# cielavenir/7bgzf

Hardware: AMD Instinct MI355X
Metric: GB/s input compressed, BGZF 64KiB blocks (higher is better)
Workload: dtype u8

## Files before the change

7bgzf_amd/csrc/hd_deflate_static.hpp:

```cpp
#pragma once
#include <type_traits>
#include "hd_device.hpp"

namespace hd {

constexpr uint32_t HD_HINT_NO_WHOLE = 1;
constexpr uint32_t HD_HINT_NO_SEG = 2;
constexpr uint32_t BESIDE_KEEP_MAX = 3;

struct DeflateArgs {
	const uint8_t *in;
	const uint64_t *in_off;
	const uint32_t *in_len;
	uint32_t nblocks;
	int frame;
	int level;
	uint8_t *out;
	uint64_t out_stride;
	uint32_t out_cap;
	uint32_t *out_len;
	uint32_t *crc;
	int32_t *status;
	const CrcTables *ct;
	uint8_t *scratch;
	uint32_t first;
	uint32_t count;
	uint32_t skip_small;
	uint32_t split_max;
	uint32_t *split_ovf;
	uint32_t seg_limit;
	uint32_t seg_bytes;
	uint32_t hint;
	const uint64_t *host_seg_off;
	const uint32_t *host_seg_len;
	uint32_t parts = 0;
	uint32_t seg_slots = 0;
	uint32_t *done_flag = nullptr, *done_count = nullptr;
	uint32_t done_epoch = 0;
	uint32_t wg = 0;
	uint32_t lat = 0;
	uint32_t wg_split = 0;
	const uint8_t *stage_in = nullptr;
	uint32_t *stalls = nullptr;
	uint32_t *ready = nullptr, *arrived = nullptr, *next = nullptr;
	uint32_t span_sub = 0;
	uint8_t *scratch_b = nullptr;
	uint32_t *emitted = nullptr;
	uint32_t take_sub = 0;
	uint32_t *poison = nullptr;
	uint32_t beside_keep = BESIDE_KEEP_MAX;
	uint32_t prime_max = 0;
	void *beside = nullptr;
};

__host__ __device__ __forceinline__ uint32_t frame_hdr_bytes(int frame)
{
	return frame == HD_FRAME_BGZF ? 18u : frame == HD_FRAME_MIGZ ? 20u : frame == HD_FRAME_ZLIB ? 2u
	     : frame == HD_FRAME_GZIP ? 10u : 0u;
}

__host__ __device__ __forceinline__ uint32_t frame_trl_bytes(int frame)
{
	return frame == HD_FRAME_ZLIB ? 4u : (frame == HD_FRAME_BGZF || frame == HD_FRAME_MIGZ || frame == HD_FRAME_GZIP) ? 8u : 0u;
}

__device__ __forceinline__ uint32_t frame_trl_field(int frame, uint32_t k, uint32_t crc, uint32_t n)
{
	const uint32_t w = k < 2 ? (frame == HD_FRAME_ZLIB ? 0u : crc) : n;
	return (w >> (16 * (k & 1))) & 0xffff;
}

__device__ __forceinline__ uint32_t frame_sfx_bytes(int frame)
{
	return frame == HD_FRAME_RAW_FLUSH ? 5u : 0u;
}

__host__ __device__ inline uint32_t seg_slots_per_block(uint32_t cap, uint32_t seg)
{
	const uint32_t full = HD_STORED_SIZE(seg) + 5u;
	return cap / full + (cap % full >= 11u ? 1u : 0u);
}

__host__ __device__ inline bool seg_coded(uint32_t len, uint32_t limit, uint32_t seg, int frame, uint64_t out_stride, uint32_t out_cap)
{
	if (!limit || len <= limit)
		return false;
	if (seg == HD_SEG_BYTES || len > HD_SEG_LIMIT)
		return true;
	uint64_t room = out_stride < out_cap ? out_stride : out_cap;
	const uint32_t S = seg_slots_per_block(room > 0x7fffffffu ? 0x7fffffffu : (uint32_t)room, seg);
	if (frame == HD_FRAME_BGZF && room > 65536)
		room = 65536;
	return HD_SEGN_COUNT(len, seg) <= S &&
	       frame_hdr_bytes(frame) + HD_SEGN_WORST((uint64_t)len, seg, frame == HD_FRAME_RAW_FLUSH) + frame_trl_bytes(frame) <= room;
}

__device__ __forceinline__ bool whole_refused(const DeflateArgs &a, uint32_t n)
{
	return a.level >= 1 && !a.seg_limit && n > HD_SEG_LIMIT;
}

__device__ __forceinline__ void refuse_member(const DeflateArgs &a, uint32_t b, uint32_t lane)
{
	if (lane == 0) {
		a.out_len[b] = 0;
		if (a.status) a.status[b] = 1;
		if (a.crc) a.crc[b] = 0;
	}
}

__device__ __forceinline__ uint32_t frame_hdr_word(int frame, uint32_t j)
{
	const bool bz = frame == HD_FRAME_BGZF, gz = frame == HD_FRAME_GZIP, zl = frame == HD_FRAME_ZLIB;
	const uint32_t w0 = zl ? 0x0000da78u : gz ? 0x00088b1fu : 0x04088b1fu;
	const uint32_t w2 = zl ? 0u : gz ? 0x00000002u : bz ? 0x0006ff00u : 0x0008ff00u;
	const uint32_t w3 = (zl || gz) ? 0u : bz ? 0x00024342u : 0x00045a4du;
	return j == 0 ? w0 : j == 1 ? 0u : j == 2 ? w2 : w3;
}

__device__ __forceinline__ uint32_t frame_hdr_byte(int frame, uint32_t o, uint32_t sizefield)
{
	const uint32_t w = o < 16 ? frame_hdr_word(frame, o >> 2) : sizefield;
	return (w >> (8 * (o & 3))) & 0xff;
}

__device__ __forceinline__ void write_stored_member(const DeflateArgs &a, uint32_t b, const uint8_t *src, uint32_t n,
						  uint32_t crc, uint32_t lane)
{
	const uint32_t hdr = frame_hdr_bytes(a.frame), trl = frame_trl_bytes(a.frame);
	const bool flush = a.frame == HD_FRAME_RAW_FLUSH;
	const uint32_t stored = HD_STORED_SIZE(n);
	const uint32_t total = hdr + stored + trl + (flush ? 5u : 0u);
	uint64_t cap = a.out_stride < a.out_cap ? a.out_stride : a.out_cap;
	if (a.frame == HD_FRAME_BGZF && cap > 65536)
		cap = 65536;
	if (total > cap) {
		if (lane == 0) {
			a.out_len[b] = 0;
			if (a.status) a.status[b] = 1;
			if (a.crc) a.crc[b] = crc;
		}
		return;
	}
	const uint32_t sizefield = a.frame == HD_FRAME_BGZF ? total - 1 : stored;
	const uint32_t nblk = n == 0 ? 1u : (n + 65534u) / 65535u;
	uint32_t *dst32 = (uint32_t *)(a.out + (uint64_t)b * a.out_stride);
	for (uint32_t j = lane; j < (total + 3) / 4; j += 64) {
		uint32_t w = 0;
		for (uint32_t k = 0; k < 4; k++) {
			uint32_t o = 4 * j + k, v = 0;
			if (o < hdr) {
				v = frame_hdr_byte(a.frame, o, sizefield);
			} else if (o < hdr + stored) {
				uint32_t q = (o - hdr) / 65540u, r = (o - hdr) - q * 65540u;
				uint32_t left = n - q * 65535u;
				uint32_t bl = left < 65535u ? left : 65535u;
				if (r == 0) v = (q + 1 == nblk && !flush) ? 1u : 0u;
				else if (r == 1) v = bl & 0xff;
				else if (r == 2) v = bl >> 8;
				else if (r == 3) v = ~bl & 0xff;
				else if (r == 4) v = (~bl >> 8) & 0xff;
				else v = src[q * 65535u + r - 5];
			} else if (o < total) {
				uint32_t t = o - hdr - stored;
				v = flush ? (t >= 3 ? 0xffu : 0u) : (frame_trl_field(a.frame, t >> 1, crc, n) >> (8 * (t & 1))) & 0xff;
			}
			w |= v << (8 * k);
		}
		dst32[j] = w;
	}
	if (lane == 0) {
		a.out_len[b] = total;
		if (a.status) a.status[b] = 0;
		if (a.crc) a.crc[b] = crc;
	}
}

__device__ __forceinline__ uint4 load_slot(const uint8_t *src, uint32_t n, uint32_t piece, uint32_t lane, bool aligned)
{
	const uint32_t o = piece * HD_PIECE + lane * 16;
	if (aligned && o + 16 <= n)
		return *(const uint4 *)(src + o);
	uint32_t w0 = 0, w1 = 0, w2 = 0, w3 = 0;
	if (o < n) {
#pragma unroll
		for (uint32_t k = 0; k < 4; k++) {
			w0 |= (o + k < n ? (uint32_t)src[o + k] : 0u) << (8 * k);
			w1 |= (o + 4 + k < n ? (uint32_t)src[o + 4 + k] : 0u) << (8 * k);
			w2 |= (o + 8 + k < n ? (uint32_t)src[o + 8 + k] : 0u) << (8 * k);
			w3 |= (o + 12 + k < n ? (uint32_t)src[o + 12 + k] : 0u) << (8 * k);
		}
	}
	return make_uint4(w0, w1, w2, w3);
}

struct SplitLayout {
	uint32_t cap_tok, max_db;
	uint64_t off_rec, off_ntok, off_hist, bytes;
};
__host__ __device__ inline SplitLayout split_layout(uint32_t max_block, bool full = false)
{
	SplitLayout l;
	l.cap_tok = full ? ((max_block + 64 + 15) & ~15u) : max_block / 4 * 3 + 128;
	l.max_db = l.cap_tok / HD_DYN_BLOCK_TOKENS + 2;
	l.off_rec = (uint64_t)l.cap_tok * 4;
	l.off_ntok = l.off_rec + 16;
	l.off_hist = (l.off_ntok + (uint64_t)l.max_db * 4 + 15) & ~(uint64_t)15;
	l.bytes = l.off_hist + (uint64_t)l.max_db * 320 * 4;
	return l;
}
__device__ __forceinline__ uint8_t *split_block(uint8_t *scratch, uint32_t max_block, uint32_t i)
{
	return scratch + (uint64_t)i * split_layout(max_block).bytes;
}
__host__ __device__ inline SplitLayout part_layout() { return split_layout(HD_LAT_PART_BYTES, true); }
__device__ __forceinline__ uint8_t *part_block(uint8_t *scratch, uint32_t i)
{
	return scratch + (uint64_t)i * part_layout().bytes;
}

template <int WIN_BITS, int HASH_BITS, bool TOK, int INTRA = 0, bool PRIMED = TOK>
__global__ __launch_bounds__(64) void k_deflate_static(DeflateArgs a)
{
	static_assert(PRIMED || !TOK, "the parse kernels are always built with the latency-mode paths");
	static_assert(!TOK || (WIN_BITS == HD_L2_WIN_BITS && HASH_BITS == HD_L2_HASH_BITS && HD_L2_MIN_LEN == HD_MIN_MATCH),
		      "the parse kernel is level 2's: its ring, its table, its minimum length");
	constexpr uint32_t W = 1u << WIN_BITS;
	constexpr uint32_t W4M = W / 4 - 1;
	constexpr uint32_t HS = HD_TABLE_ENTRIES(WIN_BITS, HASH_BITS);
	constexpr uint32_t STG = 64;
	constexpr uint32_t TOKQ = 128;
	constexpr bool K16 = TOK;

	__shared__ __attribute__((aligned(W))) uint32_t ring32[W / 4 + 4];
	__shared__ __attribute__((aligned(16))) uint16_t table[HS];
	__shared__ __attribute__((aligned(16))) uint32_t stage[TOK ? 316 : STG];
	__shared__ uint32_t tokbuf[TOKQ];
	const uint32_t ring_lds = (uint32_t)(uintptr_t)(__attribute__((address_space(3))) const void *)ring32;

	const uint32_t lane = threadIdx.x;
	const bool parted = PRIMED && TOK && a.parts != 0;
	const uint32_t b = a.first + (parted ? blockIdx.x / a.parts : blockIdx.x);
	if (b >= a.nblocks)
		return;
	const ClockStamp clk(TOK ? HD_CLK_PARSE : HD_CLK_STATIC);
	const uint8_t *src = a.in + a.in_off[b];
	uint32_t n = a.in_len[b];
	uint32_t prime = (PRIMED && HD_LAT_SEG_PRIME && a.seg_slots && b % a.seg_slots) ? HD_LAT_PRIME(HD_LAT_PRIME_BYTES, n) : 0u;
	if (parted) {
		const uint32_t o = (blockIdx.x % a.parts) * HD_LAT_PART_BYTES;
		if (o >= n)
			return;
		n = n - o < HD_LAT_PART_BYTES ? n - o : HD_LAT_PART_BYTES;
		prime = o ? HD_LAT_PRIME(o, n) : HD_LAT_PRIME(prime, n);
		src += o;
	}
	const uint8_t *const src_own = src;
	const uint32_t n_own = n;
	src -= prime;
	n += prime;
	if (TOK && !parted && (n > a.split_max || seg_coded(n_own, a.seg_limit, a.seg_bytes, a.frame, a.out_stride, a.out_cap))) {
		if (lane == 0)
			a.split_ovf[b] = 1;
		return;
	}
	if (!TOK && seg_coded(n_own, a.seg_limit, a.seg_bytes, a.frame, a.out_stride, a.out_cap))
		return;
	if (!TOK && whole_refused(a, n_own)) {
		refuse_member(a, b, lane);
		return;
	}
	const bool aligned = (((uintptr_t)src) & 15) == 0;
	uint32_t *dst32 = (uint32_t *)(a.out + (uint64_t)b * a.out_stride);
	const CrcTables *ct = a.ct;

	const uint32_t hdr = frame_hdr_bytes(a.frame), trl = frame_trl_bytes(a.frame);
	uint64_t cap64 = a.out_stride < a.out_cap ? a.out_stride : a.out_cap;
	if (a.frame == HD_FRAME_BGZF && cap64 > 65536)
		cap64 = 65536;
	const uint32_t cap = (uint32_t)cap64;
	const uint32_t stored = HD_STORED_SIZE(n_own);
	uint32_t limit = stored - 1;
	const bool flush = a.frame == HD_FRAME_RAW_FLUSH;
	const uint32_t sfx = frame_sfx_bytes(a.frame);
	bool use_static = TOK || (a.level >= 1 && cap >= hdr + trl + sfx + 2);
	if (!TOK && use_static && cap - hdr - trl - sfx < limit)
		limit = cap - hdr - trl - sfx;
	const uint32_t limit_bits = limit > 0x1fffffe0u ? 0xffffff00u : 8u * limit;

	for (uint32_t i = lane; i < HS / 8; i += 64)
		((uint4 *)table)[i] = make_uint4(0, 0, 0, 0);
	for (uint32_t i = lane; i < (TOK ? 316u : STG); i += 64)
		stage[i] = 0;
	if (!TOK && lane < 4 && hdr)
		stage[lane] = frame_hdr_word(a.frame, lane);
	const SplitLayout lay = parted ? part_layout() : split_layout(TOK ? a.split_max : 0);
	uint8_t *const rec = !TOK ? nullptr : parted ? part_block(a.scratch, blockIdx.x) : split_block(a.scratch, a.split_max, blockIdx.x);
	uint32_t *const slab = (uint32_t *)rec;
	uint32_t ntok_slab = 0, db_start = 0, ndb = 0;
	int32_t db_room = HD_DYN_BLOCK_TOKENS;

	Fn8Ident fid;
	fid.init(lane);
	Fn8Cross fcross;
	fcross.init(lane);
	uint32_t lane_k = lane + (HD_TOKEN_MATCH_TAG - (3u << 16));
	asm volatile("" : "+v"(lane_k));
	HashConsts hk;
	hk.init(HS);
	CrcLanes crc;
	crc.init(lane, n, prime);
	uint32_t filled = 0;
	uint4 pre = load_slot(src, n, 0, lane, aligned);

	uint32_t bitpos = 8 * hdr;
	uint32_t flushed = 0;
	const uint32_t paybase = 8 * hdr;

	auto put = [&](uint32_t code, uint32_t nbits, uint32_t incl, uint32_t total) {
		const uint32_t bp = bitpos + incl - nbits;
		const uint32_t sh = bp & 31, i = (bp >> 5) & (STG - 1);
		const uint64_t wide = (uint64_t)code << sh;
		atomicOr(&stage[i], (uint32_t)wide);
		atomicOr(&stage[(i + 1) & (STG - 1)], (uint32_t)(wide >> 32));
		bitpos += total;
	};
	auto drain_read = [&](uint32_t &fl) -> uint32_t {
		const uint32_t ready = (bitpos >> 5) - flushed;
		fl = flushed + lane;
		asm("" : "+v"(fl));
		uint32_t v;
		asm("" : "=v"(v));
		if (lane < ready) {
			const uint32_t i = fl & (STG - 1);
			v = stage[i];
			stage[i] = 0;
		}
		return v;
	};
	auto drain_store = [&](uint32_t fl, uint32_t v) {
		const uint32_t ready = (bitpos >> 5) - flushed;
		if (lane < ready)
			dst32[fl] = v;
		flushed = bitpos >> 5;
	};
	auto drain = [&]() {
		uint32_t fl;
		const uint32_t v = drain_read(fl);
		drain_store(fl, v);
	};
	auto crc_then_prefetch = [&](uint32_t piece, uint4 v) {
		crc.fold(ct, piece, piece * HD_PIECE + lane * 16 + 16 <= n && piece * HD_PIECE + lane * 16 >= prime, v);
		asm volatile("" : "+v"(crc.s) : : "memory");
		if (filled < n)
			pre = load_slot(src, n, piece + 1, lane, aligned);
	};
	auto fill_piece = [&]() {
		const uint32_t piece = filled / HD_PIECE;
		const uint4 v = pre;
		filled += HD_PIECE;
		const uint32_t ro = (piece * HD_PIECE) & (W - 1);
		((uint4 *)ring32)[ro / 16 + lane] = v;
		if (ro == 0 && lane == 0)
			((uint4 *)ring32)[W / 16] = v;
		crc_then_prefetch(piece, v);
	};
	struct Fetched {
		uint32_t v, vh, c;
	};
	constexpr bool OWN_AHEAD = false;
	struct Own {
		uint32_t w0, w1, w2;
	};
	auto own = [&](uint32_t S_) -> Own {
		const uint32_t *w = &ring32[((S_ + lane) >> 2) & W4M];
		Own o = { w[0], w[1], w[2] };
		return o;
	};
	Own o1 = { 0, 0, 0 };
	auto fetch = [&](auto inner_tag, uint32_t S_) -> Fetched {
		constexpr bool INNER = decltype(inner_tag)::value;
		Fetched f;
		const uint32_t p = S_ + lane;
		const uint32_t *w = &ring32[(p >> 2) & W4M];
		uint32_t w0, w1, w2;
		if (OWN_AHEAD && S_ >= 128) {
			w0 = o1.w0;
			w1 = o1.w1;
			w2 = o1.w2;
		} else {
			w0 = w[0];
			w1 = w[1];
			w2 = w[2];
		}
		f.v = __builtin_amdgcn_alignbyte(w1, w0, p & 3);
		f.vh = __builtin_amdgcn_alignbyte(w2, w1, p & 3);
		const bool can = INNER || p + HD_MIN_MATCH <= n;
		const uint32_t ha = hash_slot_addr(f.v, hk);
		uint16_t *const slot = (uint16_t *)((uint8_t *)table + (can ? ha : 0u));
		const uint16_t mine = (uint16_t)(p + 1);
		const uint32_t e = *slot;
		if (can)
			*slot = mine;
		if (INNER) {
			f.c = e;
		} else {
			const uint32_t back = (p + 1 - e) & 0xffffu;
			f.c = (can && e && back) ? p + 1 - back : 0u;
		}
		if (INTRA) {
			const uint32_t d = intra_step_distance<INTRA>(f.v, lane);
			f.c = (can && d) ? p + 1 - d : f.c;
		}
		return f;
	};
	struct Probed {
		uint32_t c0, c1, c2;
		uint32_t spare[10];
	};
	auto probe = [&](uint32_t c, uint32_t p) -> Probed {
		Probed q = {};
		const uint32_t *w = &ring32[((c - 1) >> 2) & W4M];
		q.c0 = w[0];
		q.c1 = w[1];
		q.c2 = w[2];
		return q;
	};

	uint32_t qhead = 0, qtail = 0;
	uint32_t Q0 = 0, qn = 0;
	uint32_t Qp = 0;
	uint64_t qpm = 0;
	auto queue_settle = [&]() {
		Q0 = sel(qpm, Qp, Q0);
		qpm = 0;
	};
	auto count_symbol = [&](uint32_t c) {
		atomicAdd(&stage[c], 1u);
	};
	auto emit_tokens = [&](uint32_t count, uint32_t tq) -> bool {
		uint32_t t = tq;
		if (TOK) {
			t = tokbuf[(qhead + lane) & (TOKQ - 1)];
			qhead += count;
		}
		if (!use_static)
			return false;
		if (TOK) {
			if (ntok_slab + count > lay.cap_tok)
				return use_static = false;
			if (lane < count) {
				slab[ntok_slab + lane] = t;
				if (t & HD_TOKEN_MATCH) {
					uint32_t ls, leb, lev, ds, deb, dev;
					len_slot(((t >> 16) & 0xff) + 3, ls, leb, lev);
					off_slot((t & 0xffff) + 1, ds, deb, dev);
					count_symbol(257 + ls);
					count_symbol(286 + ds);
				} else {
					count_symbol(t & 0xff);
				}
			}
			ntok_slab += count;
			return true;
		}
		const uint64_t mmask = __ballot((int32_t)t < 0);
		const uint64_t vmask = count >= 64 ? ~0ull : (1ull << (count & 63)) - 1;
		uint32_t e0 = ct->SL[sel(mmask, (t >> 16) & 0x1ff, t & 0xff)];
		uint32_t ds, deb, dev;
		off_slot((t & 0xffff) + 1, ds, deb, dev);
		uint32_t dpart = (__brev(ds) >> 27) | (dev << 5);
		asm volatile("" : "+v"(dpart), "+v"(deb) : : "memory");
		uint32_t fl;
		const uint32_t dv = drain_read(fl);
		asm volatile("" : "+v"(e0) : : "memory");
		drain_store(fl, dv);
		const uint32_t nb0 = e0 >> 16;
		const uint32_t code = sel(vmask, sel(mmask, (e0 & 0xffff) | (dpart << nb0), e0 & 0xffff), 0u);
		const uint32_t nbits = sel(vmask, sel(mmask, nb0 + 5 + deb, nb0), 0u);
		const uint32_t incl = wave_incl_scan<true>(nbits);
		const uint32_t total = readlane(incl, 63);
		if ((bitpos - paybase) + total + 7 > limit_bits)
			return use_static = false;
		put(code, nbits, incl, total);
		return true;
	};

	if (!TOK)
		put(lane == 0 ? (flush ? 2u : 3u) : 0u, lane == 0 ? 3u : 0u, 3u, 3u);

	Fetched f0 = { 0, 0, 0 }, f1 = { 0, 0, 0 };
	Probed q0 = {};
	if (use_static && n) {
		fill_piece();
		f0 = fetch(std::false_type{}, 0);
		q0 = probe(f0.c, lane);
		f1 = fetch(std::false_type{}, 64);
		if (OWN_AHEAD)
			o1 = own(128);
	}
	uint32_t carry = 0;
	auto step = [&](auto inner_tag, auto nofill_tag, auto room258_tag, uint32_t S) -> bool {
		constexpr bool INNER = decltype(inner_tag)::value;
		constexpr bool NOFILL = decltype(nofill_tag)::value;
		constexpr bool ROOM258 = decltype(room258_tag)::value;
		if (!NOFILL && filled < n && filled < S + HD_LOOKAHEAD)
			fill_piece();
		const uint32_t lo = filled > W ? filled - W : 0;
		const uint32_t lanes = INNER ? 64u : (n - S < 64 ? n - S : 64);

		const Fetched fc = f0;
		const Probed qc = q0;
		f0 = f1;
		q0 = probe(f1.c, S + 64 + lane);
		f1 = fetch(inner_tag, S + 128);
		if (OWN_AHEAD)
			o1 = own(S + 192);
		if (!TOK)
			queue_settle();

		const uint64_t lanem = (INNER || lanes == 64) ? ~0ull : (1ull << (lanes & 63)) - 1;
		constexpr bool GROUP = !TOK && INNER && ROOM258;
		const uint32_t p = S + (GROUP ? lane_k : lane);
		const uint32_t cv0 = fc.v, cvh0 = fc.vh;
		const uint32_t room = n - p;
		const uint32_t c = fc.c, cp = c - 1;
		const uint32_t cv = __builtin_amdgcn_alignbyte(qc.c1, qc.c0, cp);
		const uint32_t cvh = __builtin_amdgcn_alignbyte(qc.c2, qc.c1, cp);
		const uint32_t x = cvh ^ cvh0;
		const uint64_t xm = __ballot(cvh == cvh0);
		const uint32_t len8 = sel(xm, 8u, 4u + ((uint32_t)__builtin_ctz(x) >> 3));
		uint64_t okm = __ballot((int32_t)cp >= (int32_t)lo) & __ballot(cv == cv0);
		const uint32_t mylen = INNER ? len8 : (len8 < room ? len8 : room);
		if (!INNER)
			okm &= __ballot(p + HD_MIN_MATCH <= n);

		if (carry >= lanes) {
			carry -= lanes;
			return true;
		}

		const uint64_t capmask = INNER ? (okm & xm) : (okm & xm & __ballot(room > 8));
		const uint32_t jump8 = sel(okm, mylen, 1u);
		uint32_t lenv = jump8;
		const uint64_t livem = ~0ull << carry;
		const uint32_t mw_base = GROUP ? p - c : (p + (HD_TOKEN_MATCH_TAG - (3u << 16) - 1u)) - cp;
		const uint32_t lit = cv0 & 0xff;
		uint32_t len16 = 8;
		const bool k16_step = K16 && capmask != 0;
		if (k16_step) {
			const uint32_t *wp = &ring32[(p >> 2) & W4M], *wc = &ring32[(cp >> 2) & W4M];
			const uint32_t c2 = qc.c2;
			const uint32_t p2 = wp[2], p3 = wp[3], p4 = wp[4];
			const uint32_t c3 = wc[3], c4 = wc[4];
			const uint32_t xa = __builtin_amdgcn_alignbyte(p3, p2, p & 3) ^ __builtin_amdgcn_alignbyte(c3, c2, cp);
			const uint32_t xb = __builtin_amdgcn_alignbyte(p4, p3, p & 3) ^ __builtin_amdgcn_alignbyte(c4, c3, cp);
			uint32_t fa, fb;
			asm("v_ffbl_b32 %0, %1" : "=v"(fa) : "v"(xa));
			asm("v_ffbl_b32 %0, %1" : "=v"(fb) : "v"(xb));
			const uint32_t ka = (fa >> 3) < 4 ? (fa >> 3) : 4u, kb = (fb >> 3) < 4 ? (fb >> 3) : 4u;
			len16 = 8 + ka + (ka >> 2) * kb;
			if (!INNER)
				len16 = len16 < room ? len16 : room;
		}
		uint64_t k8m = 0, par = 0, contm = 0;
		uint32_t jumpA = jump8, jumpW = jump8;
		if (k16_step) {
			k8m = capmask & __ballot(len16 == 16);
			const uint64_t capk = capmask & ~k8m & __ballot(len16 != 8);
			par = capk;
			if (capk & (capk << 8)) {
#pragma unroll
				for (int i = 0; i < 7; i++)
					par = capk & ~(par << 8);
			}
			contm = (par << 8) & lanem;
			const uint32_t kc = (uint32_t)__builtin_amdgcn_ds_bpermute((int)((lane - 8) << 2), (int)(len16 - 8));
			jumpW = sel(capk, len16, jump8);
			jumpA = sel(contm, kc, jump8);
			lenv = jumpW;
		}
		uint64_t starts;
		{
			Fn8 f;
			f.lo = sel(livem, jumpA + 0x0200ffffu, 0x02010000u);
			f.hi = 0x06050403u;
			const uint32_t w0 = fn8_scan_state0(f, fid, fcross);
			starts = livem & ~(__ballot((w0 & 0xff) != 0) << 1);
		}
		uint64_t v = 0;
		if (K16) {
			uint64_t pend = ~0ull;
			for (;;) {
				v = starts & contm & ((starts & par) << 8);
				const uint64_t ev = starts & (k8m | contm) & ~v & pend;
				if (!ev)
					break;
				const uint32_t m = (uint32_t)__ffsll((unsigned long long)ev) - 1;
				uint32_t len;
				if ((k8m >> m) & 1) {
					const uint32_t pm = S + m;
					const uint32_t dm = pm + 1 - readlane(c, m);
					const uint32_t maxlen = n - pm < HD_MAX_MATCH ? n - pm : HD_MAX_MATCH;
					uint32_t t0, t1, k;
					len = 16;
					asm volatile("Lhd_ext_%=:\n\t"
					     "v_add_u32 %[t0], %[len], %[vb]\n\t"
					     "v_add_u32 %[t1], %[ndm], %[t0]\n\t"
					     "v_and_or_b32 %[t0], %[t0], %[msk], %[rb]\n\t"
					     "v_and_or_b32 %[t1], %[t1], %[msk], %[rb]\n\t"
					     "ds_read_u8 %[t0], %[t0]\n\t"
					     "ds_read_u8 %[t1], %[t1]\n\t"
					     "s_waitcnt lgkmcnt(0)\n\t"
					     "v_cmp_ne_u16 vcc, %[t0], %[t1]\n\t"
					     "s_cbranch_vccnz Lhd_ext_hit_%=\n\t"
					     "s_add_u32 %[len], %[len], 64\n\t"
					     "s_cmp_lt_u32 %[len], %[maxlen]\n\t"
					     "s_cbranch_scc1 Lhd_ext_%=\n\t"
					     "s_branch Lhd_ext_done_%=\n"
					     "Lhd_ext_hit_%=:\n\t"
					     "s_ff1_i32_b64 %[k], vcc\n\t"
					     "s_add_u32 %[len], %[len], %[k]\n"
					     "Lhd_ext_done_%=:"
					     : [len] "+s"(len), [t0] "=&v"(t0), [t1] "=&v"(t1), [k] "=&s"(k)
					     : [vb] "v"(pm + lane), [ndm] "s"(0u - dm), [msk] "s"(W - 1), [rb] "v"(ring_lds), [maxlen] "s"(maxlen)
					     : "vcc", "scc", "memory");
					len = len < maxlen ? len : maxlen;
					asm("s_mov_b32 m0, %2\n\ts_nop 0\n\tv_writelane_b32 %0, %1, m0" : "+v"(lenv) : "s"(len), "s"(m));
				} else {
					len = readlane(jumpW, m);
				}
				uint64_t fresh = 0;
				uint32_t xq = m + (uint32_t)__builtin_amdgcn_readfirstlane((int)len), hop;
				asm volatile("s_cmp_gt_u32 %0, 63\n\t"
					     "s_cbranch_scc1 Lhd_rethread_done_%=\n"
					     "Lhd_rethread_%=:\n\t"
					     "s_bitcmp1_b64 %3, %0\n\t"
					     "s_cbranch_scc1 Lhd_rethread_done_%=\n\t"
					     "s_bitset1_b64 %1, %0\n\t"
					     "v_readlane_b32 %2, %4, %0\n\t"
					     "s_add_u32 %0, %0, %2\n\t"
					     "s_cmp_lt_u32 %0, 64\n\t"
					     "s_cbranch_scc1 Lhd_rethread_%=\n"
					     "Lhd_rethread_done_%=:"
					     : "+s"(xq), "+s"(fresh), "=&s"(hop)
					     : "s"(starts & ~contm), "v"(jumpW)
					     : "scc");
				const uint32_t xe = xq < 64 ? xq : 64;
				uint64_t gone;
				asm("s_bfm_b64 %0, %1, %2" : "=s"(gone) : "s"(xe - m - 1), "s"(m + 1));
				starts = (starts & ~gone) | fresh;
				pend = ~1ull << m;
			}
		} else {
			uint64_t todo = capmask;
			uint64_t cm = starts & todo;
			if (cm) {
				uint32_t t0, t1, x, cq, len, k;
				uint64_t fresh;
#define HD_L1_EVENTS(CLAMP)                                                                  \
	"s_ff1_i32_b64 m0, %[cm]\n\t"                                                        \
	"s_bitset0_b64 %[todo], m0\n\t"                                                      \
	"v_readlane_b32 %[cq], %[cp], m0\n\t"                                                \
	"s_add_u32 %[x], m0, 2\n"                                                            \
	"Lhd_ext_%=:\n\t"                                                                    \
	"v_add_u32 %[t0], %[x], %[p]\n\t"                                                    \
	"v_add_u32 %[t1], %[cq], %[lane]\n\t"                                                \
	"v_and_b32 %[t0], %[wm], %[t0]\n\t"                                                  \
	"v_and_b32 %[t1], %[wm], %[t1]\n\t"                                                  \
	"ds_read_u8 %[t0], %[t0]\n\t"                                                        \
	"ds_read_u8 %[t1], %[t1] offset:2\n\t"                                               \
	"s_waitcnt lgkmcnt(0)\n\t"                                                           \
	"v_cmp_ne_u16 vcc, %[t0], %[t1]\n\t"                                                 \
	"s_cbranch_vccnz Lhd_ext_hit_%=\n\t"                                                 \
	"s_add_u32 %[x], %[x], 64\n\t"                                                       \
	"s_add_u32 %[cq], %[cq], 64\n\t"                                                     \
	"s_sub_u32 %[len], %[x], m0\n\t"                                                     \
	"s_cmp_lt_u32 %[len], 258\n\t"                                                       \
	"s_cbranch_scc1 Lhd_ext_%=\n\t"                                                      \
	"s_branch Lhd_ext_len_%=\n"                                                          \
	"Lhd_ext_hit_%=:\n\t"                                                                \
	"s_ff1_i32_b64 %[k], vcc\n\t"                                                        \
	"s_add_u32 %[x], %[x], %[k]\n\t"                                                     \
	"s_sub_u32 %[len], %[x], m0\n"                                                       \
	"Lhd_ext_len_%=:\n\t"                                                                \
	CLAMP                                                                                \
	"v_writelane_b32 %[lenv], %[len], m0\n\t"                                            \
	"s_mov_b64 %[fresh], 0\n\t"                                                          \
	"s_cmp_gt_u32 %[x], 63\n\t"                                                          \
	"s_cbranch_scc1 Lhd_rethread_out_%=\n"                                               \
	"Lhd_rethread_%=:\n\t"                                                               \
	"s_bitcmp1_b64 %[starts], %[x]\n\t"                                                  \
	"s_cbranch_scc1 Lhd_rethread_done_%=\n\t"                                            \
	"s_bitset1_b64 %[fresh], %[x]\n\t"                                                   \
	"v_readlane_b32 %[k], %[lenv], %[x]\n\t"                                             \
	"s_add_u32 %[x], %[x], %[k]\n\t"                                                     \
	"s_cmp_lt_u32 %[x], 64\n\t"                                                          \
	"s_cbranch_scc1 Lhd_rethread_%=\n"                                                   \
	"Lhd_rethread_out_%=:\n\t"                                                           \
	"s_movk_i32 %[x], 64\n"                                                              \
	"Lhd_rethread_done_%=:\n\t"                                                          \
	"s_add_u32 %[k], m0, 1\n\t"                                                          \
	"s_sub_u32 %[len], %[x], %[k]\n\t"                                                   \
	"s_bfm_b64 %[cm], %[len], %[k]\n\t"                                                  \
	"s_andn2_b64 %[starts], %[starts], %[cm]\n\t"                                        \
	"s_or_b64 %[starts], %[starts], %[fresh]\n"                                          \
	"s_and_b64 %[cm], %[starts], %[todo]"
				do {
					if (ROOM258)
						asm volatile(HD_L1_EVENTS("")
						  : [starts] "+s"(starts), [todo] "+s"(todo), [cm] "+s"(cm), [lenv] "+v"(lenv), [t0] "=&v"(t0), [t1] "=&v"(t1),
						    [x] "=&s"(x), [cq] "=&s"(cq), [len] "=&s"(len), [k] "=&s"(k), [fresh] "=&s"(fresh)
						  : [cp] "v"(cp), [p] "v"(p), [lane] "v"(lane), [wm] "n"(W - 1)
						  : "vcc", "scc", "memory");
					else
						asm volatile(HD_L1_EVENTS("s_sub_u32 %[k], %[left], m0\n\t"
								       "s_min_u32 %[k], %[k], 258\n\t"
								       "s_min_u32 %[len], %[len], %[k]\n\t"
								       "s_add_u32 %[x], %[len], m0\n\t")
						  : [starts] "+s"(starts), [todo] "+s"(todo), [cm] "+s"(cm), [lenv] "+v"(lenv), [t0] "=&v"(t0), [t1] "=&v"(t1),
						    [x] "=&s"(x), [cq] "=&s"(cq), [len] "=&s"(len), [k] "=&s"(k), [fresh] "=&s"(fresh)
						  : [cp] "v"(cp), [p] "v"(p), [lane] "v"(lane), [wm] "n"(W - 1), [left] "s"(n - S)
						  : "vcc", "scc", "memory");
				} while (cm);
#undef HD_L1_EVENTS
			}
		}
		const uint64_t real = starts & ~v;
		const uint32_t last = K16 ? 63 - (uint32_t)__clzll((long long)real) : ~(uint32_t)__builtin_clzll(real);
		const uint32_t E = last + readlane(lenv, last);
		const uint64_t tm = starts & lanem & ~v;
		const uint64_t mm = tm & okm;
		if (!(INNER || lanes == 64))
			carry = 0;
		else if (K16)
			asm("s_max_u32 %0, %1, 64\n\ts_sub_u32 %0, %0, 64" : "=s"(carry) : "s"(E) : "scc");
		else
			asm("s_max_i32 %0, %1, 0" : "=s"(carry) : "s"(E) : "scc");

		const uint32_t tw = sel(mm, (lenv << 16) + mw_base, lit);
		if (TOK) {
			const uint32_t rank = __builtin_amdgcn_mbcnt_hi((uint32_t)(tm >> 32), __builtin_amdgcn_mbcnt_lo((uint32_t)tm, 0));
			const uint32_t qslot = (qtail + rank) & (TOKQ - 1);
			if ((tm >> lane) & 1)
				tokbuf[qslot] = tw;
			qtail += (uint32_t)__popcll(tm);
			db_room -= (int32_t)__popcll(tm);
			if (qtail - qhead >= 64)
				emit_tokens(64, 0);
		} else {
			const uint32_t R = queue_push(tm, qn, tw);
			uint64_t newm;
			asm("s_lshl_b64 %0, -1, %1" : "=s"(newm) : "s"(qn) : "scc");
			Qp = R;
			qpm = newm;
			qn += (uint32_t)__popcll(tm);
			if (qn >= 64) {
				emit_tokens(64, sel(newm, R, Q0));
				qpm = ~0ull;
				qn -= 64;
			}
		}
		return use_static;
	};
	const bool small = n <= 65536;
	auto close_deflate_block = [&]() {
		uint32_t *h = (uint32_t *)(rec + lay.off_hist) + ndb * 320;
		for (uint32_t i = lane; i < 320; i += 64) {
			const uint32_t j = i < 286 ? i : i - 2;
			const bool used = i < 286 || (i >= 288 && i < 318);
			h[i] = used ? stage[j] : 0u;
		}
		for (uint32_t i = lane; i < 316u; i += 64)
			stage[i] = 0;
		if (lane == 0)
			((uint32_t *)(rec + lay.off_ntok))[ndb] = ntok_slab - db_start;
		db_start = ntok_slab;
		db_room = HD_DYN_BLOCK_TOKENS;
		ndb++;
	};
	auto step_boundary = [&](auto inner_tag, uint32_t S) -> bool {
		constexpr bool INNER = decltype(inner_tag)::value;
		if (TOK && db_room <= 0 && use_static && (INNER || S + 64 < n)) {
			if (qtail != qhead && !emit_tokens(qtail - qhead, 0))
				return false;
			close_deflate_block();
		}
		return use_static;
	};
	uint32_t S = 0;
	clk.mark(0);
	for (; S < prime && use_static; S += 64) {
		if (filled < n && filled < S + HD_LOOKAHEAD)
			fill_piece();
		f0 = f1;
		q0 = probe(f1.c, S + 64 + lane);
		f1 = fetch(std::false_type{}, S + 128);
		if (OWN_AHEAD)
			o1 = own(S + 192);
	}
	while (S < n && use_static) {
		if (small && filled < n && filled < S + HD_LOOKAHEAD && S + 15 * 64 + 63 + HD_MAX_MATCH <= n) {
			fill_piece();
#pragma unroll 1
			for (uint32_t g = 0; g < 4 && use_static; g++) {
#pragma unroll
				for (uint32_t u = 0; u < 4; u++) {
					step(std::true_type{}, std::true_type{}, std::true_type{}, S);
					step_boundary(std::true_type{}, S);
					S += 64;
				}
			}
			continue;
		}
		const bool ok_step = (small && S + 192 + 8 <= n) ? step(std::true_type{}, std::false_type{}, std::false_type{}, S)
								  : step(std::false_type{}, std::false_type{}, std::false_type{}, S);
		if (!ok_step || !step_boundary(std::false_type{}, S))
			break;
		S += 64;
	}
	if (TOK && use_static && qtail != qhead)
		emit_tokens(qtail - qhead, 0);
	if (!TOK)
		queue_settle();
	if (!TOK && use_static && qn)
		emit_tokens(uniform(qn), Q0);
	clk.mark(1);

	while (filled < n) {
		const uint32_t piece = filled / HD_PIECE;
		const uint4 pv = pre;
		filled += HD_PIECE;
		if (filled < n)
			pre = load_slot(src, n, piece + 1, lane, aligned);
		crc.fold(ct, piece, piece * HD_PIECE + lane * 16 + 16 <= n && piece * HD_PIECE + lane * 16 >= prime, pv);
	}
	const uint32_t crcv = crc.finish(ct, lane, n, src + (n & ~15u));
	clk.mark(2);

	if (TOK) {
		if (use_static)
			close_deflate_block();
		if (lane == 0) {
			uint32_t *m = (uint32_t *)(rec + lay.off_rec);
			m[0] = use_static ? ndb : 0xffffffffu;
			m[1] = crcv;
			if (!parted)
				a.split_ovf[b] = use_static ? 0u : 1u;
		}
		return;
	}
	if (use_static && (uint64_t)(bitpos - paybase) + 7 > 8ull * limit)
		use_static = false;
	if (!use_static) {
		write_stored_member(a, b, src_own, n_own, crcv, lane);
		return;
	}

	bitpos += 7;
	drain();
	if (flush) {
		bitpos = (bitpos + 3 + 7) & ~7u;
		uint32_t tcode = 0, nb = 0;
		if (lane < 2) {
			tcode = lane ? 0xffffu : 0u;
			nb = 16;
		}
		const uint32_t incl = wave_incl_scan<true>(nb);
		put(tcode, nb, incl, 32);
	}
	bitpos = (bitpos + 7) & ~7u;
	const uint32_t paylen = (bitpos - paybase) >> 3;
	if (trl) {
		uint32_t tcode = 0, nb = 0;
		if (lane < trl / 2) {
			tcode = frame_trl_field(a.frame, lane, crcv, n_own);
			nb = 16;
		}
		const uint32_t incl = wave_incl_scan<true>(nb);
		put(tcode, nb, incl, 8 * trl);
	}
	for (uint32_t i = flushed + lane; i < ((bitpos + 31) >> 5); i += 64)
		dst32[i] = stage[i & (STG - 1)];
	if (lane == 0) {
		const uint32_t total = hdr + paylen + trl;
		if (a.frame == HD_FRAME_BGZF)
			*(uint16_t *)((uint8_t *)dst32 + 16) = (uint16_t)(total - 1);
		else if (a.frame == HD_FRAME_MIGZ)
			dst32[4] = paylen;
		a.out_len[b] = total;
		if (a.status) a.status[b] = 0;
		if (a.crc) a.crc[b] = crcv;
	}
}

}
```

7bgzf_amd/csrc/hd_device.hpp:

```cpp
#pragma once
#include <hip/hip_runtime.h>
#include <stdint.h>
#include "../../include/hipdeflate_params.h"

namespace hd {

struct CrcTables {
	uint32_t T[4][256];
	uint32_t B[4][256];
	uint32_t B16[4][256];
	uint32_t BL[4][256];
	uint32_t T16[16][256];
	uint32_t K[64];
	uint32_t SL[512];
	uint32_t P2[24][4][256];
	uint32_t SM[3][16][4][256];
};

#ifdef HD_CLOCK_STAMPS
__device__ unsigned long long g_clk[4][4];
__device__ unsigned long long g_clk_mark[16];
struct ClockStamp {
	unsigned long long t0, r0;
	int k;
	__device__ __forceinline__ void mark(int i) const
	{
		unsigned long long t;
		asm volatile("s_memtime %0\n\ts_waitcnt lgkmcnt(0)" : "=s"(t)::"memory");
		if (threadIdx.x == 0) {
			atomicAdd(&g_clk_mark[i], t - t0);
			atomicAdd(&g_clk_mark[8 + i], 1ull);
		}
	}
	__device__ __forceinline__ ClockStamp(int kernel) : k(kernel)
	{
		asm volatile("s_memrealtime %0\n\ts_memtime %1\n\ts_waitcnt lgkmcnt(0)" : "=s"(r0), "=s"(t0)::"memory");
	}
	__device__ __forceinline__ ~ClockStamp()
	{
		unsigned long long t1, r1;
		asm volatile("s_memtime %0\n\ts_memrealtime %1\n\ts_waitcnt lgkmcnt(0)" : "=s"(t1), "=s"(r1)::"memory");
		if (threadIdx.x == 0) {
			atomicAdd(&g_clk[k][0], t1 - t0);
			atomicAdd(&g_clk[k][1], r1 - r0);
			atomicAdd(&g_clk[k][2], 1ull);
		}
	}
};
#else
struct ClockStamp {
	__device__ __forceinline__ ClockStamp(int) {}
	__device__ __forceinline__ void mark(int) const {}
};
#endif
enum { HD_CLK_STATIC = 0, HD_CLK_DYNAMIC = 1, HD_CLK_INFLATE = 2, HD_CLK_PARSE = 3 };

template <int CTRL, int ROW_MASK, int BANK_MASK, bool BC = false>
__device__ __forceinline__ uint32_t dpp0(uint32_t v)
{
	return (uint32_t)__builtin_amdgcn_update_dpp(0, (int)v, CTRL, ROW_MASK, BANK_MASK, BC);
}

template <bool BC = false>
__device__ __forceinline__ uint32_t wave_incl_scan(uint32_t x)
{
	uint32_t v = x;
	v += dpp0<0x111, 0xf, 0xf, BC>(x);
	v += dpp0<0x112, 0xf, 0xf, BC>(x);
	v += dpp0<0x113, 0xf, 0xf, BC>(x);
	v += dpp0<0x114, 0xf, 0xe, BC>(v);
	v += dpp0<0x118, 0xf, 0xc, BC>(v);
	v += dpp0<0x142, 0xa, 0xf, BC>(v);
	v += dpp0<0x143, 0xc, 0xf, BC>(v);
	return v;
}

struct Fn8 {
	uint32_t lo, hi;
};

struct Fn8Ident {
	uint32_t lo[4], hi[4];
	__device__ __forceinline__ void init(uint32_t lane)
	{
		const uint32_t r = lane & 15;
		const bool none[4] = { r < 1, r < 2, r < 4, r < 8 };
#pragma unroll
		for (int k = 0; k < 4; k++)
			lo[k] = none[k] ? 0x03020100u : 0u;
		const uint32_t k0 = r < 1 ? 0u : 1u;
		const uint32_t k1 = r < 2 ? 0u : r < 3 ? 1u : 2u;
		const uint32_t k2 = r < 4 ? 0u : r < 7 ? r - 3 : 4u;
		hi[0] = 0x07060504u - 0x01010101u * k0;
		hi[1] = 0x07060504u - 0x01010101u * k1;
		hi[2] = 0x07060504u - 0x01010101u * k2;
		hi[3] = none[3] ? 0x07060504u : 0u;
	}
};

template <int CTRL, int ROW_MASK>
__device__ __forceinline__ Fn8 fn8_dpp(Fn8 v, uint32_t id_lo, uint32_t id_hi)
{
	Fn8 r;
	r.lo = dpp0<CTRL, ROW_MASK, 0xf>(v.lo) | id_lo;
	r.hi = dpp0<CTRL, ROW_MASK, 0xf>(v.hi) | id_hi;
	return r;
}

template <int CTRL, int ROW_MASK>
__device__ __forceinline__ Fn8 fn8_dpp_lo(Fn8 v, uint32_t id_lo, uint32_t sel_hi)
{
	Fn8 r;
	r.lo = dpp0<CTRL, ROW_MASK, 0xf>(v.lo) | id_lo;
	r.hi = sel_hi;
	return r;
}

__device__ __forceinline__ Fn8 fn8_compose(Fn8 then, Fn8 first)
{
	Fn8 r;
	r.lo = __builtin_amdgcn_perm(then.hi, then.lo, first.lo);
	r.hi = __builtin_amdgcn_perm(then.hi, then.lo, first.hi);
	return r;
}

struct Fn8Cross {
	uint32_t lo15, hi15, lo31;
	__device__ __forceinline__ void init(uint32_t lane)
	{
		lo15 = (lane & 16) ? 0u : 0x03020100u;
		hi15 = (lane & 16) ? 0u : 0x07060504u;
		lo31 = lane < 32 ? 0x03020100u : 0u;
		asm volatile("" : "+v"(lo15), "+v"(hi15), "+v"(lo31));
	}
};

__device__ __forceinline__ uint32_t fn8_scan_state0(Fn8 w, const Fn8Ident &id, const Fn8Cross &x)
{
	w = fn8_compose(w, fn8_dpp_lo<0x111, 0xf>(w, id.lo[0], id.hi[0]));
	w = fn8_compose(w, fn8_dpp_lo<0x112, 0xf>(w, id.lo[1], id.hi[1]));
	w = fn8_compose(w, fn8_dpp_lo<0x114, 0xf>(w, id.lo[2], id.hi[2]));
	w = fn8_compose(w, fn8_dpp<0x118, 0xf>(w, id.lo[3], id.hi[3]));
	uint32_t rl, rh, out;
	asm("s_nop 1\n\t"
	    "v_mov_b32_dpp %[xl], %[wl] row_bcast:15 row_mask:0xa bank_mask:0xf\n\t"
	    "v_mov_b32_dpp %[xh], %[wh] row_bcast:15 row_mask:0xa bank_mask:0xf\n\t"
	    "v_perm_b32 %[rl], %[wh], %[wl], %[xl]\n\t"
	    "v_perm_b32 %[rh], %[wh], %[wl], %[xh]\n\t"
	    "s_nop 0\n\t"
	    "v_mov_b32_dpp %[xm], %[rl] row_bcast:31 row_mask:0xc bank_mask:0xf\n\t"
	    "v_perm_b32 %[out], %[rh], %[rl], %[xm]"
	    : [rl] "=&v"(rl), [rh] "=&v"(rh), [out] "=&v"(out)
	    : [xl] "v"(x.lo15), [xh] "v"(x.hi15), [xm] "v"(x.lo31), [wl] "v"(w.lo), [wh] "v"(w.hi));
	return out;
}

template <int CTRL, int ROW_MASK>
__device__ __forceinline__ Fn8 fn8_dpp_seeded(Fn8 v)
{
	Fn8 r;
	r.lo = (uint32_t)__builtin_amdgcn_update_dpp((int)0x03020100, (int)v.lo, CTRL, ROW_MASK, 0xf, false);
	r.hi = (uint32_t)__builtin_amdgcn_update_dpp((int)0x07060504, (int)v.hi, CTRL, ROW_MASK, 0xf, false);
	return r;
}

__device__ __forceinline__ Fn8 fn8_scan(Fn8 w)
{
	w = fn8_compose(w, fn8_dpp_seeded<0x111, 0xf>(w));
	w = fn8_compose(w, fn8_dpp_seeded<0x112, 0xf>(w));
	w = fn8_compose(w, fn8_dpp_seeded<0x114, 0xf>(w));
	w = fn8_compose(w, fn8_dpp_seeded<0x118, 0xf>(w));
	w = fn8_compose(w, fn8_dpp_seeded<0x142, 0xa>(w));
	w = fn8_compose(w, fn8_dpp_seeded<0x143, 0xc>(w));
	return w;
}

__device__ __forceinline__ Fn8 fn8_make(bool live, uint32_t a)
{
	Fn8 f;
	f.lo = live ? (0x02010000u | a) : 0x03020100u;
	f.hi = live ? 0x06050403u : 0x07060504u;
	return f;
}

__device__ __forceinline__ uint32_t wave_xor_reduce(uint32_t v)
{
	for (int o = 32; o > 0; o >>= 1)
		v ^= (uint32_t)__shfl_xor((int)v, o, 64);
	return v;
}

__device__ __forceinline__ uint32_t readlane(uint32_t v, uint32_t l)
{
	return (uint32_t)__builtin_amdgcn_readlane((int)v, (int)l);
}

__device__ __forceinline__ uint32_t uniform(uint32_t v)
{
	return (uint32_t)__builtin_amdgcn_readfirstlane((int)v);
}

__device__ __forceinline__ uint32_t sel(uint64_t mask, uint32_t a, uint32_t b)
{
	uint32_t d;
	asm("v_cndmask_b32_e64 %0, %1, %2, %3" : "=v"(d) : "v"(b), "v"(a), "s"(mask));
	return d;
}

__device__ __forceinline__ uint32_t queue_push(uint64_t tm, uint32_t q, uint32_t tw)
{
	const uint32_t rank = __builtin_amdgcn_mbcnt_hi((uint32_t)(tm >> 32), __builtin_amdgcn_mbcnt_lo((uint32_t)tm, 0));
	return (uint32_t)__builtin_amdgcn_ds_permute((int)((rank + q) << 2), (int)tw);
}

struct HashConsts {
	uint32_t k1, k2, e2, m;
	__device__ __forceinline__ void init(uint32_t entries)
	{
		k1 = HD_HASH_K1;
		k2 = HD_HASH_K2;
		e2 = 2 * entries;
		m = 0xfffeu;
	}
};
__device__ __forceinline__ uint32_t hash_slot_addr(uint32_t v, const HashConsts &k)
{
	uint32_t t1, t, x, a;
	asm("v_mul_u32_u24_sdwa %0, %1, %2 dst_sel:DWORD dst_unused:UNUSED_PAD src0_sel:WORD_1 src1_sel:DWORD"
	    : "=v"(t1) : "v"(v), "v"(k.k2));
	asm("v_mad_u32_u24 %0, %1, %2, %3" : "=v"(t) : "v"(v), "v"(k.k1), "v"(t1));
	asm("v_mul_u32_u24_sdwa %0, %1, %2 dst_sel:DWORD dst_unused:UNUSED_PAD src0_sel:WORD_1 src1_sel:DWORD"
	    : "=v"(x) : "v"(t), "v"(k.e2));
	asm("v_and_b32_sdwa %0, %1, %2 dst_sel:DWORD dst_unused:UNUSED_PAD src0_sel:WORD_1 src1_sel:DWORD"
	    : "=v"(a) : "v"(x), "v"(k.m));
	return a;
}

struct HashConsts6 {
	uint32_t k1, k2, k3, e4, m;
	__device__ __forceinline__ void init(uint32_t buckets)
	{
		k1 = HD_HASH_K1;
		k2 = HD_HASH_K2;
		k3 = HD_HASH_K3;
		e4 = 4 * buckets;
		m = 0xfffcu;
	}
};
__device__ __forceinline__ uint32_t hash_slot_addr6(uint32_t v, uint32_t vh, const HashConsts6 &k)
{
	uint32_t t1, t2, t, x, a;
	asm("v_mul_u32_u24_sdwa %0, %1, %2 dst_sel:DWORD dst_unused:UNUSED_PAD src0_sel:WORD_1 src1_sel:DWORD"
	    : "=v"(t1) : "v"(v), "v"(k.k2));
	asm("v_mul_u32_u24_sdwa %0, %1, %2 dst_sel:DWORD dst_unused:UNUSED_PAD src0_sel:WORD_0 src1_sel:DWORD"
	    : "=v"(t2) : "v"(vh), "v"(k.k3));
	asm("v_mad_u32_u24 %0, %1, %2, %3" : "=v"(t) : "v"(v), "v"(k.k1), "v"(t1));
	t += t2;
	asm("v_mul_u32_u24_sdwa %0, %1, %2 dst_sel:DWORD dst_unused:UNUSED_PAD src0_sel:WORD_1 src1_sel:DWORD"
	    : "=v"(x) : "v"(t), "v"(k.e4));
	asm("v_and_b32_sdwa %0, %1, %2 dst_sel:DWORD dst_unused:UNUSED_PAD src0_sel:WORD_1 src1_sel:DWORD"
	    : "=v"(a) : "v"(x), "v"(k.m));
	return a;
}

__device__ __forceinline__ uint32_t crc_step4(const CrcTables *ct, uint32_t s, uint32_t d)
{
	s ^= d;
	return ct->T[3][s & 0xff] ^ ct->T[2][(s >> 8) & 0xff] ^ ct->T[1][(s >> 16) & 0xff] ^ ct->T[0][s >> 24];
}

__device__ __forceinline__ uint32_t crc_shift(const uint32_t (*Z)[256], uint32_t s)
{
	return Z[0][s & 0xff] ^ Z[1][(s >> 8) & 0xff] ^ Z[2][(s >> 16) & 0xff] ^ Z[3][s >> 24];
}

__device__ __forceinline__ uint32_t crc_byte(const CrcTables *ct, uint32_t s, uint32_t b)
{
	return ct->T[0][(s ^ b) & 0xff] ^ (s >> 8);
}

__device__ __forceinline__ uint32_t gf_mul(uint32_t a, uint32_t b)
{
	uint32_t p = 0;
#pragma unroll 4
	for (int i = 0; i < 32; i++) {
		p ^= b & (0u - ((a >> (31 - i)) & 1u));
		b = (b >> 1) ^ (0xEDB88320u & (0u - (b & 1u)));
	}
	return p;
}

__device__ inline uint32_t crc_append_bytes(const CrcTables *ct, uint32_t s, uint64_t n)
{
	for (int j = 0; n && j < 24; j++, n >>= 1)
		if (n & 1)
			s = crc_shift(ct->P2[j], s);
	for (; n; n--)
		s = crc_shift(ct->P2[23], crc_shift(ct->P2[23], s));
	return s;
}

struct CrcLanes {
	uint32_t s;
	__device__ __forceinline__ void init(uint32_t lane, uint32_t n, uint32_t first = 0)
	{
		s = (lane == first / 16 && n >= 16) ? 0xffffffffu : 0u;
	}
	template <bool CHAIN = false>
	__device__ __forceinline__ void fold(const CrcTables *ct, uint32_t piece, bool full, uint4 v)
	{
		if (CHAIN) {
			if (full) {
				uint32_t t = s;
				if (piece)
					t = ct->BL[0][s & 0xff] ^ ct->BL[1][(s >> 8) & 0xff] ^ ct->BL[2][(s >> 16) & 0xff] ^ ct->BL[3][s >> 24];
				t = crc_step4(ct, t, v.x);
				t = crc_step4(ct, t, v.y);
				t = crc_step4(ct, t, v.z);
				s = crc_step4(ct, t, v.w);
			}
			return;
		}
		if (full) {
			const uint32_t (*Z)[256] = piece ? ct->B : ct->B16;
			uint32_t t = Z[0][s & 0xff] ^ Z[1][(s >> 8) & 0xff] ^ Z[2][(s >> 16) & 0xff] ^ Z[3][s >> 24];
			const uint32_t w[4] = { v.x, v.y, v.z, v.w };
#pragma unroll
			for (int k = 0; k < 4; k++)
				t ^= ct->T16[15 - 4 * k][w[k] & 0xff] ^ ct->T16[14 - 4 * k][(w[k] >> 8) & 0xff] ^
				     ct->T16[13 - 4 * k][(w[k] >> 16) & 0xff] ^ ct->T16[12 - 4 * k][w[k] >> 24];
			s = t;
		}
	}
	__device__ __forceinline__ uint32_t finish(const CrcTables *ct, uint32_t lane, uint32_t n,
						    const uint8_t *tail)
	{
		uint32_t n16 = n >> 4;
		uint32_t acc = 0;
		if (lane < n16) {
			uint32_t jl = lane + 64u * ((n16 - 1 - lane) >> 6);
			acc = gf_mul(ct->K[n16 - 1 - jl], s);
		}
		acc = wave_xor_reduce(acc);
		if (n16 == 0)
			acc = 0xffffffffu;
		for (uint32_t i = n16 << 4; i < n; i++)
			acc = crc_byte(ct, acc, tail[i - (n16 << 4)]);
		return ~acc;
	}
};

template <int DIST>
__device__ __forceinline__ uint32_t intra_step_distance(uint32_t v, uint32_t lane)
{
	uint32_t sh = v, best = 0;
#pragma unroll
	for (int d = 1; d <= DIST; d++) {
		sh = (uint32_t)__builtin_amdgcn_update_dpp(0, (int)sh, 0x138 , 0xf, 0xf, false);
		best = (best == 0 && sh == v && lane >= (uint32_t)d) ? (uint32_t)d : best;
	}
	return best;
}

struct AdlerLanes {
	uint32_t s1, s2;
	__device__ __forceinline__ void init() { s1 = s2 = 0; }
	__device__ __forceinline__ void fold(uint32_t piece, uint32_t lane, uint4 v)
	{
		uint32_t sum = __builtin_amdgcn_sad_u8(v.x, 0u, 0u);
		sum = __builtin_amdgcn_sad_u8(v.y, 0u, sum);
		sum = __builtin_amdgcn_sad_u8(v.z, 0u, sum);
		sum = __builtin_amdgcn_sad_u8(v.w, 0u, sum);
		uint32_t ws = __builtin_amdgcn_udot4(v.x, 0x03020100u, 0u, false);
		ws = __builtin_amdgcn_udot4(v.y, 0x07060504u, ws, false);
		ws = __builtin_amdgcn_udot4(v.z, 0x0b0a0908u, ws, false);
		ws = __builtin_amdgcn_udot4(v.w, 0x0f0e0d0cu, ws, false);
		const uint32_t g = (piece * HD_PIECE + lane * 16) % 65521u;
		s1 += sum;
		s2 = (s2 + g * sum + ws) % 65521u;
	}
	__device__ __forceinline__ uint32_t finish(uint32_t n)
	{
		const uint32_t S1 = readlane(wave_incl_scan(s1 % 65521u), 63) % 65521u;
		const uint32_t S2 = readlane(wave_incl_scan(s2), 63) % 65521u;
		const uint32_t nm = n % 65521u;
		const uint32_t a = (1u + S1) % 65521u;
		const uint32_t b = (nm + (uint32_t)(((uint64_t)nm * S1) % 65521u) + 65521u - S2) % 65521u;
		return (b << 16) | a;
	}
};

__device__ __forceinline__ void len_slot(uint32_t len, uint32_t &sym, uint32_t &eb, uint32_t &ev)
{
	uint32_t l = len - 3;
	uint32_t e = (l < 8) ? 0 : (29 - __clz(l));
	sym = (l < 8) ? l : (4 + 4 * e + ((l >> e) & 3));
	eb = e;
	ev = l & ((1u << e) - 1);
	if (l == 255) { sym = 28; eb = 0; ev = 0; }
}

__device__ __forceinline__ void off_slot(uint32_t off, uint32_t &sym, uint32_t &eb, uint32_t &ev)
{
	uint32_t d = off - 1;
	uint32_t e = (d < 4) ? 0 : (30 - __clz(d));
	sym = (d < 4) ? d : (2 * e + 2 + ((d >> e) & 1));
	eb = e;
	ev = d & ((1u << e) - 1);
}

}
```

Baseline: 410.0.

## Software-pipeline static Huffman table gather across match-finding steps

Result: no change. 411.7 (median of 6 runs) (+0.4%).

```diff
diff --git a/7bgzf_amd/csrc/hd_deflate_static.hpp b/7bgzf_amd/csrc/hd_deflate_static.hpp
--- a/7bgzf_amd/csrc/hd_deflate_static.hpp
+++ b/7bgzf_amd/csrc/hd_deflate_static.hpp
@@ -325,9 +325,9 @@
 		atomicOr(&stage[(i + 1) & (STG - 1)], (uint32_t)(wide >> 32));
 		bitpos += total;
 	};
-	auto drain_read = [&](uint32_t &fl) -> uint32_t {
+	auto drain = [&]() {
 		const uint32_t ready = (bitpos >> 5) - flushed;
-		fl = flushed + lane;
+		uint32_t fl = flushed + lane;
 		asm("" : "+v"(fl));
 		uint32_t v;
 		asm("" : "=v"(v));
@@ -335,19 +335,9 @@
 			const uint32_t i = fl & (STG - 1);
 			v = stage[i];
 			stage[i] = 0;
-		}
-		return v;
-	};
-	auto drain_store = [&](uint32_t fl, uint32_t v) {
-		const uint32_t ready = (bitpos >> 5) - flushed;
-		if (lane < ready)
 			dst32[fl] = v;
+		}
 		flushed = bitpos >> 5;
-	};
-	auto drain = [&]() {
-		uint32_t fl;
-		const uint32_t v = drain_read(fl);
-		drain_store(fl, v);
 	};
 	auto crc_then_prefetch = [&](uint32_t piece, uint4 v) {
 		crc.fold(ct, piece, piece * HD_PIECE + lane * 16 + 16 <= n && piece * HD_PIECE + lane * 16 >= prime, v);
@@ -464,26 +454,57 @@
 			ntok_slab += count;
 			return true;
 		}
-		const uint64_t mmask = __ballot((int32_t)t < 0);
-		const uint64_t vmask = count >= 64 ? ~0ull : (1ull << (count & 63)) - 1;
-		uint32_t e0 = ct->SL[sel(mmask, (t >> 16) & 0x1ff, t & 0xff)];
+		return false;
+	};
+	uint32_t pend_t = 0, pend_e = 0;
+	uint32_t pass_limit = limit_bits;
+	uint64_t pend_m = 0;
+	unsigned long long pend_clk = clk.span_open();
+	auto pass_finish = [&](auto full_tag, uint64_t vmask) {
+		constexpr bool FULL = decltype(full_tag)::value;
+		const uint32_t t = pend_t;
+		const uint64_t mmask = pend_m;
+		const unsigned long long tw = clk.span_open();
+		asm volatile("s_waitcnt vmcnt(0)" : "+v"(pend_e) : : "memory");
+		const uint32_t e0 = pend_e;
+		clk.span_close(HD_SPAN_GATHER_WAIT, tw);
+		clk.span_close(HD_SPAN_GATHER, pend_clk);
+		clk.span_close(HD_SPAN_EMPTY, clk.span_open());
+		drain();
 		uint32_t ds, deb, dev;
 		off_slot((t & 0xffff) + 1, ds, deb, dev);
-		uint32_t dpart = (__brev(ds) >> 27) | (dev << 5);
-		asm volatile("" : "+v"(dpart), "+v"(deb) : : "memory");
-		uint32_t fl;
-		const uint32_t dv = drain_read(fl);
-		asm volatile("" : "+v"(e0) : : "memory");
-		drain_store(fl, dv);
+		const uint32_t dpart = (__brev(ds) >> 27) | (dev << 5);
 		const uint32_t nb0 = e0 >> 16;
-		const uint32_t code = sel(vmask, sel(mmask, (e0 & 0xffff) | (dpart << nb0), e0 & 0xffff), 0u);
-		const uint32_t nbits = sel(vmask, sel(mmask, nb0 + 5 + deb, nb0), 0u);
+		const uint32_t code_all = sel(mmask, (e0 & 0xffff) | (dpart << nb0), e0 & 0xffff);
+		const uint32_t nbits_all = sel(mmask, nb0 + 5 + deb, nb0);
+		const uint32_t code = FULL ? code_all : sel(vmask, code_all, 0u);
+		const uint32_t nbits = FULL ? nbits_all : sel(vmask, nbits_all, 0u);
 		const uint32_t incl = wave_incl_scan<true>(nbits);
 		const uint32_t total = readlane(incl, 63);
-		if ((bitpos - paybase) + total + 7 > limit_bits)
-			return use_static = false;
-		put(code, nbits, incl, total);
-		return true;
+		if ((bitpos - paybase) + total + 7 > pass_limit) {
+			use_static = false;
+			pass_limit = 0;
+		} else {
+			put(code, nbits, incl, total);
+		}
+	};
+	uint32_t gather_due;
+	asm volatile("s_mov_b32 %0, 0" : "=s"(gather_due));
+	auto pass_take = [&](uint32_t tq) {
+		const unsigned long long th = clk.span_open();
+		pend_t = tq;
+		asm volatile("" : "+v"(pend_t) : : "memory");
+		clk.span_close(HD_SPAN_PUSH_WAIT, th);
+	};
+	auto pass_gather = [&]() {
+		pend_m = __ballot((int32_t)pend_t < 0);
+		pend_clk = clk.span_open();
+		const uint32_t word = sel(pend_m, (pend_t >> 14) & 0x7fc, (pend_t << 2) & 0x3fc);
+		asm volatile("global_load_dword %0, %1, %2" : "+&v"(pend_e) : "v"(word), "s"(ct->SL) : "memory");
+		asm volatile("s_mov_b32 %0, 0" : "=s"(gather_due));
+	};
+	auto gather_landed = [&]() {
+		asm volatile("s_waitcnt vmcnt(0)" : "+v"(pend_e) : : "memory");
 	};
 
 	if (!TOK)
@@ -518,6 +539,11 @@
 			o1 = own(S + 192);
 		if (!TOK)
 			queue_settle();
+		if (!TOK && gather_due) {
+			pass_gather();
+			if (!(INNER && ROOM258))
+				gather_landed();
+		}
 
 		const uint64_t lanem = (INNER || lanes == 64) ? ~0ull : (1ull << (lanes & 63)) - 1;
 		constexpr bool GROUP = !TOK && INNER && ROOM258;
@@ -535,9 +561,10 @@
 		if (!INNER)
 			okm &= __ballot(p + HD_MIN_MATCH <= n);
 
+		const auto scan_and_push = [&]() {
 		if (carry >= lanes) {
 			carry -= lanes;
-			return true;
+			return;
 		}
 
 		const uint64_t capmask = INNER ? (okm & xm) : (okm & xm & __ballot(room > 8));
@@ -755,11 +782,15 @@
 			Qp = R;
 			qpm = newm;
 			qn += (uint32_t)__popcll(tm);
-			if (qn >= 64) {
-				emit_tokens(64, sel(newm, R, Q0));
-				qpm = ~0ull;
-				qn -= 64;
-			}
+		}
+		};
+		scan_and_push();
+		if (!TOK && qn >= 64) {
+			pass_finish(std::true_type{}, ~0ull);
+			pass_take(sel(qpm, Qp, Q0));
+			asm volatile("s_mov_b32 %0, 1" : "=s"(gather_due));
+			qpm = ~0ull;
+			qn -= 64;
 		}
 		return use_static;
 	};
@@ -811,6 +842,8 @@
 					S += 64;
 				}
 			}
+			if (!TOK)
+				gather_landed();
 			continue;
 		}
 		const bool ok_step = (small && S + 192 + 8 <= n) ? step(std::true_type{}, std::false_type{}, std::false_type{}, S)
@@ -823,8 +856,17 @@
 		emit_tokens(qtail - qhead, 0);
 	if (!TOK)
 		queue_settle();
-	if (!TOK && use_static && qn)
-		emit_tokens(uniform(qn), Q0);
+	if (!TOK && use_static) {
+		if (gather_due)
+			pass_gather();
+		pass_finish(std::true_type{}, ~0ull);
+		if (use_static && qn) {
+			const uint32_t count = uniform(qn);
+			pass_take(Q0);
+			pass_gather();
+			pass_finish(std::false_type{}, (1ull << (count & 63)) - 1);
+		}
+	}
 	clk.mark(1);
 
 	while (filled < n) {
diff --git a/7bgzf_amd/csrc/hd_device.hpp b/7bgzf_amd/csrc/hd_device.hpp
--- a/7bgzf_amd/csrc/hd_device.hpp
+++ b/7bgzf_amd/csrc/hd_device.hpp
@@ -23,6 +23,7 @@
 struct ClockStamp {
 	unsigned long long t0, r0;
 	int k;
+	mutable unsigned long long span_sum[5] = { 0, 0, 0, 0, 0 }, span_n[5] = { 0, 0, 0, 0, 0 };
 	__device__ __forceinline__ void mark(int i) const
 	{
 		unsigned long long t;
@@ -32,6 +33,19 @@
 			atomicAdd(&g_clk_mark[8 + i], 1ull);
 		}
 	}
+	__device__ __forceinline__ unsigned long long span_open() const
+	{
+		unsigned long long t;
+		asm volatile("s_memtime %0" : "=s"(t)::"memory");
+		return t;
+	}
+	__device__ __forceinline__ void span_close(int i, unsigned long long opened) const
+	{
+		unsigned long long t;
+		asm volatile("s_memtime %0\n\ts_waitcnt lgkmcnt(0)" : "=s"(t), "+s"(opened)::"memory");
+		span_sum[i - 3] += t - opened;
+		span_n[i - 3] += 1;
+	}
 	__device__ __forceinline__ ClockStamp(int kernel) : k(kernel)
 	{
 		asm volatile("s_memrealtime %0\n\ts_memtime %1\n\ts_waitcnt lgkmcnt(0)" : "=s"(r0), "=s"(t0)::"memory");
@@ -44,6 +58,11 @@
 			atomicAdd(&g_clk[k][0], t1 - t0);
 			atomicAdd(&g_clk[k][1], r1 - r0);
 			atomicAdd(&g_clk[k][2], 1ull);
+			for (int i = 0; i < 5; i++)
+				if (span_n[i]) {
+					atomicAdd(&g_clk_mark[3 + i], span_sum[i]);
+					atomicAdd(&g_clk_mark[8 + 3 + i], span_n[i]);
+				}
 		}
 	}
 };
@@ -51,8 +70,11 @@
 struct ClockStamp {
 	__device__ __forceinline__ ClockStamp(int) {}
 	__device__ __forceinline__ void mark(int) const {}
+	__device__ __forceinline__ unsigned long long span_open() const { return 0; }
+	__device__ __forceinline__ void span_close(int, unsigned long long) const {}
 };
 #endif
+enum { HD_SPAN_PUSH_WAIT = 3, HD_SPAN_GATHER = 4, HD_SPAN_GATHER_WAIT = 5, HD_SPAN_EMPTY = 6 };
 enum { HD_CLK_STATIC = 0, HD_CLK_DYNAMIC = 1, HD_CLK_INFLATE = 2, HD_CLK_PARSE = 3 };
 
 template <int CTRL, int ROW_MASK, int BANK_MASK, bool BC = false>
```
